# reonaledo/Multi-modality-Self-supervision

Hardware: AMD Instinct MI355X
Metric: image-text pairs/sec pretraining step, BERT-base seq512 (higher is better)
Workload: dtype f16

## Files before the change

### include/medvill.h

```cpp
#ifndef MEDVILL_H_
#define MEDVILL_H_

#include <stddef.h>
#include <stdint.h>

#ifdef __cplusplus
extern "C" {
#endif

#define MV_ABI_VERSION 6

enum { MV_F32 = 0, MV_BF16 = 1, MV_F16 = 2 };

enum {
  MV_OK = 0,
  MV_E_ARG = -1,
  MV_E_SHAPE = -2,
  MV_E_DTYPE = -3,
  MV_E_WORKSPACE = -4,
  MV_E_NO_RCCL = -5,
  MV_E_COMM_BASE = -1000
};

enum {
// ... 27 lines not shown

size_t mv_gemm_workspace_bytes(int dtype, int ta, int tb, int M, int N, int K);
size_t mv_workspace_bytes(int hidden, int intermediate, int vocab, int img_hidden, int max_rows, int max_label_rows, int max_regions);

typedef struct mv_group_problem {
  const void* A; const void* B; void* C;
  int lda, ldb, ldc;
  int No, Ko, rows;
} mv_group_problem;
size_t mv_gemm_grouped_table_bytes(int count);
int mv_gemm_grouped_fill(int dtype, int count, const mv_group_problem* problems, int n_blocks, void* table_host, size_t table_bytes);
size_t mv_gemm_grouped_workspace_bytes(const void* table_host);
int mv_gemm_grouped_decode(const void* table_host, int unit, int* out);
int mv_gemm_grouped_tn(int dtype, int count, const void* table_host, const void* table_dev, float* ws, size_t ws_bytes,
                       int accumulate, const float* alpha_dev, void* stream);

int mv_mask_pack(const int64_t* mask, int mask_ndim, int B, int L,
                 uint32_t* bits, uint8_t* tileinfo, void* stream);

int mv_mask_build(const int32_t* desc, int B, int L, uint32_t* bits, uint8_t* tileinfo, void* stream);

int mv_mlm_draws(unsigned long long key, int B, int S, int vocab, float* u, int32_t* rnd, void* stream);
int mv_mlm_corrupt(const int64_t* ids, const int32_t* lengths, const float* u, const int32_t* rnd, const int32_t* family,
                   int B, int N, int S, int64_t* input_txt, int64_t* segment, int64_t* txt_labels, int32_t* n_ids,
                   int32_t* desc, int32_t* counts, int32_t* label_rows, int32_t* label_ids, int32_t* n_labels, void* stream);

int mv_mask_verify_host(const int64_t* mask, int mask_ndim, const int32_t* desc, int B, int L, int threads, long long* first_mismatch);

int mv_comm_unique_id(void* id128);
int mv_comm_init(void** comm_out, int rank, int world, const void* id128);
// ... 142 lines not shown
```

### multi-modality-self-supervision_amd/_lib.py

```python
from __future__ import annotations

import ctypes as C
import os

import torch

HERE = os.path.dirname(os.path.abspath(__file__))
LIB_PATH = os.environ.get("MV_LIB_PATH") or os.path.join(HERE, "libmedvill_hip.so")
DBG_LIB_PATH = os.environ.get("MV_DBG_LIB_PATH") or (LIB_PATH[:-3] + "_dbg.so")

MV_F32, MV_BF16, MV_F16 = 0, 1, 2
EPI_NONE, EPI_BIAS, EPI_BIAS_GELU, EPI_BIAS_RES, EPI_DGELU, EPI_RES, EPI_BIAS_TANH, EPI_BIAS_GELU_D, EPI_MUL, EPI_BIAS_RELU, EPI_BIAS_RES_RELU = range(11)
_ERR = {-1: "MV_E_ARG (null pointer / bad size)", -2: "MV_E_SHAPE (unsupported shape or alignment)",
        -3: "MV_E_DTYPE", -4: "MV_E_WORKSPACE (workspace too small)", -5: "MV_E_NO_RCCL (librccl could not be loaded)"}

vp, i32, i64, f32, sz, u64, f64 = C.c_void_p, C.c_int, C.c_longlong, C.c_float, C.c_size_t, C.c_ulonglong, C.c_double

PROTOTYPES = {
    "mv_abi_version": [],
    "mv_build_info": [],
    "mv_stream_create_cumask": [vp, i32, C.POINTER(C.c_void_p)],
    "mv_stream_destroy": [vp],
    "mv_comm_unique_id": [vp],
    "mv_comm_init": [C.POINTER(C.c_void_p), i32, i32, vp],
    "mv_comm_allreduce_async": [vp, vp, sz, i32, vp],
    "mv_comm_wait": [vp, vp],
    "mv_comm_destroy": [vp],
    "mv_gemm": [i32, i32, i32, i32, i32, i32, vp, i32, vp, i32, vp, i32, i32, vp, i32, vp, i32, i32, vp, i32, vp, i32, i32,
                i32, vp, sz, i32, f32, u64, vp, vp, vp],
    "mv_gemm_workspace_bytes": [i32, i32, i32, i32, i32, i32],
    "mv_workspace_bytes": [i32, i32, i32, i32, i32, i32, i32],
    "mv_gemm_grouped_table_bytes": [i32],
    "mv_gemm_grouped_fill": [i32, i32, vp, i32, vp, sz],
    "mv_gemm_grouped_workspace_bytes": [vp],
    "mv_gemm_grouped_decode": [vp, i32, C.POINTER(C.c_int)],
    "mv_gemm_grouped_tn": [i32, i32, vp, vp, vp, sz, i32, vp, vp],
    "mv_mask_pack": [vp, i32, i32, i32, vp, vp, vp],
    "mv_mask_build": [vp, i32, i32, vp, vp, vp],
    "mv_mask_verify_host": [vp, i32, vp, i32, i32, i32, C.POINTER(C.c_longlong)],
    "mv_mlm_draws": [u64, i32, i32, i32, vp, vp, vp],
    "mv_mlm_corrupt": [vp, vp, vp, vp, vp, i32, i32, i32, vp, vp, vp, vp, vp, vp, vp, vp, vp, vp],
    "mv_pack_plan": [vp, i32, i32, vp, vp, vp, vp],
    "mv_tail_perm": [vp, i32, i32, vp, i32, vp, vp, vp, vp, vp],
    "mv_attn_fwd": [i32, vp, vp, vp, vp, vp, vp, i32, i32, i32, i32, f32, vp, vp, i32, vp, vp],
    "mv_attn_dropmask": [f32, u64, i32, i32, i32, vp, vp, vp],
    "mv_attn_bwd": [i32, vp, vp, vp, vp, vp, vp, vp, vp, i32, i32, i32, i32, f32, vp, vp, i32, vp, vp],
    "mv_layernorm_fwd": [i32, vp, i32, vp, vp, vp, vp, vp, vp, i32, i32, f32, vp],
    "mv_layernorm_bwd": [i32, vp, vp, i32, vp, vp, vp, vp, vp, vp, vp, i32, i32, vp, f32, u64, vp, vp],
    "mv_embed_fwd": [i32, vp, vp, vp, vp, vp, vp, vp, vp, vp, vp, vp, vp, vp, vp, vp, vp, i32, i32, i32, i32, i32, i32, f32, f32, f32,
                     u64, vp, i32, vp],
    "mv_embed_bwd": [i32, vp, vp, vp, vp, vp, vp, vp, vp, vp, vp, vp, vp, vp, vp, vp, vp, i32, i32, i32, i32, i32, i32, i32, f32, f32,
# ... 26 lines not shown
    "mv_bce_fwd_bwd": [vp, i32, vp, vp, i32, i32, vp, vp, i32, i32, vp, f32, vp, vp, vp, vp],
    "mv_rows_mul": [i32, vp, i32, vp, vp, i32, vp, i32, i32, vp, i32, vp],
    "mv_tensor_sqnorms": [vp, sz, vp, i32, vp, i32, vp, vp, vp],
    "mv_bce_multilabel": [vp, i32, vp, vp, i32, i32, vp, vp, i32, i32, vp, f32, vp, vp, vp, vp],
    "mv_bertadam_step": [vp, vp, vp, vp, vp, vp, sz, vp, i32, vp, i32, vp, f64, f64, f64, f32, f32, f32, i32, i32, f64, i32, vp, vp],
    "mv_lm_loss_fwd": [vp, i32, i32, i32, vp, vp, i32, f64, vp, vp, vp, vp],
    "mv_lm_loss_select": [vp, vp, vp, vp, i32, i32, i32, vp, vp, vp, vp],
    "mv_lm_loss_bwd": [vp, i32, i32, i32, vp, vp, vp, vp, i32, f64, vp, vp, vp, vp, vp, vp, i32, i32, vp],
    "mv_pair_draws": [u64, u64, i32, i32, vp, vp],
    "mv_pair_negatives": [vp, i32, i32, vp, u64, u64, vp, i32, vp, vp, vp],
    "mv_pair_assemble": [vp, vp, i32, vp, i32, i32, vp, vp, i32, i32, i32, i32, vp, vp, vp, vp, vp, vp, vp],
    "mv_rank_groups": [vp, vp, i32, i32, vp, i32, vp, vp, vp, vp, vp],
}
DEBUG_PROTOTYPES = {"mv_debug_set_knob": [i32, i32], "mv_debug_get_knob": [i32]}
_RESTYPE = {"mv_build_info": C.c_char_p, "mv_gemm_workspace_bytes": C.c_size_t, "mv_workspace_bytes": C.c_size_t,
            "mv_gemm_grouped_table_bytes": C.c_size_t, "mv_gemm_grouped_workspace_bytes": C.c_size_t}
ABI_VERSION = 6

KNOBS = {"impl": (0, 0), "gemm_force": (1, 0), "gemm_nj": (2, 0), "gemm_dbg": (3, 0), "attn_planes": (4, 16), "persistent_cus": (5, 0),
         "rowops_variant": (6, 0), "attn_order": (7, 0), "attn_fwd": (8, 0), "gemm_rounds": (9, 1)}

_lib = None
_dbg = None
_knobs = {k: d for k, (_, d) in KNOBS.items()}


def _open(path, protos):
    lib = C.CDLL(path)
    for name, args in protos.items():
        fn = getattr(lib, name)
        fn.argtypes = args
# ... 89 lines not shown
```

### multi-modality-self-supervision_amd/csrc/mv_gemm.hip

```cpp
#include "mv_gemm_common.h"
#include "mv_gemm_group.h"

#define GT_BM 128
#define GT_BN 128
#define GT_BK 64
#define GT_STAGE_BYTES 32768

template <bool TR>
__device__ __forceinline__ void stage_load(u32x4 (&reg)[4], __amdgpu_buffer_rsrc_t rs, unsigned bytes, int ld,
                                           int row0, int rows_total, int k0, int kend, int tid) {
#pragma unroll
  for (int i = 0; i < 4; ++i) {
    const int idx = tid + 256 * i;
    unsigned off;
    bool ok;
    if (!TR) {
      const int r = idx >> 3, ch = idx & 7;
      const int gr = row0 + r, gk = k0 + ch * 8;
      ok = (gr < rows_total) && (gk < kend);
      off = ((unsigned)gr * (unsigned)ld + (unsigned)gk) * 2u;
    } else {
      const int kr = idx >> 4, ch = idx & 15;
      const int gk = k0 + kr, gc = row0 + ch * 8;
      ok = (gk < kend) && (gc < rows_total);
// ... 539 lines not shown
  if (n_blocks < 0) return MV_E_ARG;
  return mv_group_fill(dtype, count, problems, n_blocks > 0 ? n_blocks : grouped_blocks(), table_host, table_bytes);
}

extern "C" size_t mv_gemm_grouped_workspace_bytes(const void* table_host) { return mv_group_workspace_bytes(table_host); }

extern "C" int mv_gemm_grouped_decode(const void* table_host, int unit, int* out) {
  if (!table_host || !out) return MV_E_ARG;
  const MvGroupHeader& h = *(const MvGroupHeader*)table_host;
  if (h.magic != MV_GROUP_MAGIC || unit < 0 || unit >= h.direct + h.tail * h.split) return MV_E_ARG;
  const MvGroupUnit d = mv_group_decode(h, (const MvGroupEntry*)((const char*)table_host + sizeof(MvGroupHeader)), unit);
  out[0] = d.problem; out[1] = d.m0; out[2] = d.n0; out[3] = d.kbeg; out[4] = d.kend; out[5] = d.slice; out[6] = d.tile;
  return MV_OK;
}

extern "C" int mv_gemm_grouped_tn(int dtype, int count, const void* table_host, const void* table_dev, float* ws, size_t ws_bytes,
                                  int accumulate, const float* alpha_dev, void* stream_) {
  if (!table_host || !table_dev || count <= 0) return MV_E_ARG;
  const int rc = mv_group_check_table(dtype, count, table_host);
  if (rc != MV_OK) return rc;
  if (g_mv_impl != 0) return MV_E_DTYPE;
  if (((uintptr_t)table_dev) & 15) return MV_E_SHAPE;
  const MvGroupHeader& h = *(const MvGroupHeader*)table_host;
  const size_t need = mv_group_workspace_bytes(table_host);
  if (need > 0 && (!ws || ws_bytes < need || (((uintptr_t)ws) & 15))) return MV_E_WORKSPACE;
  GroupArgs ga;
  ga.table = table_dev; ga.ws = ws; ga.alpha = alpha_dev; ga.accumulate = accumulate;
  const int n_blk = h.n_blocks < grouped_blocks() ? h.n_blocks : grouped_blocks();
  return mv_launch_ring_tn_grouped(h, ga, dtype == MV_F16, n_blk, (hipStream_t)stream_);
}

extern "C" int mv_conv2d(int dtype, const void* x, const void* w, void* y, int y_dtype, int B, int H, int W, int C, int O, int kh, int kw,
                         int stride, int pad, const float* bias, int epi, const void* R, int r_dtype, void* stream_) {
  hipStream_t stream = (hipStream_t)stream_;
  if (!x || !w || !y || B <= 0 || H <= 0 || W <= 0 || C <= 0 || O <= 0 || kh <= 0 || kw <= 0 || stride <= 0 || pad < 0) return MV_E_ARG;
  if (dtype != MV_BF16 || g_mv_impl != 0) return MV_E_DTYPE;
  if (y_dtype != MV_F32 && y_dtype != MV_BF16) return MV_E_DTYPE;
  if (epi != MV_EPI_NONE && epi != MV_EPI_BIAS && epi != MV_EPI_BIAS_RELU && epi != MV_EPI_BIAS_RES_RELU) return MV_E_ARG;
  if (epi != MV_EPI_NONE && !bias) return MV_E_ARG;
  if (epi == MV_EPI_BIAS_RES_RELU && (!R || (r_dtype != MV_F32 && r_dtype != MV_BF16))) return MV_E_ARG;
  if ((C & 7) || (C & (C - 1)) || (O & 3)) return MV_E_SHAPE;
  const int Ho = (H + 2 * pad - kh) / stride + 1, Wo = (W + 2 * pad - kw) / stride + 1;
  if (Ho <= 0 || Wo <= 0) return MV_E_SHAPE;
  const long long rows = (long long)B * Ho * Wo;
// ... 28 lines not shown
```

### multi-modality-self-supervision_amd/csrc/mv_gemm_group.h

```cpp
#pragma once
#include <stddef.h>
#include <stdint.h>
#include "../../include/medvill.h"

#if defined(__HIPCC__)
#include <hip/hip_runtime.h>
#define MV_HD __host__ __device__ __forceinline__
#else
#define MV_HD inline
#endif

#define MV_GROUP_MAGIC 0x4d564754
#define MV_GROUP_MAX_PROBLEMS 256
#define MV_GROUP_MAX_SPLIT 8
#define MV_GROUP_TILE 256
#define MV_GROUP_BK 64

struct MvGroupHeader {
  int magic, count, dtype, n_blocks;
  int units;
  int direct;
  int tail;
  int split;
  int pad[8];
};
struct MvGroupEntry {
  const void* A; const void* B; void* C;
  int lda, ldb, ldc;
  int M, N, K;
  unsigned bytesA, bytesB;
  int unit0;
  int kchunk;
};
struct GroupArgs {
  const void* table;
  float* ws;
  const float* alpha;
  int accumulate;
};
static_assert(sizeof(MvGroupHeader) == 64 && sizeof(MvGroupEntry) == 64, "table layout");

MV_HD int mv_group_tiles(int M, int N) { return ((M + MV_GROUP_TILE - 1) / MV_GROUP_TILE) * ((N + MV_GROUP_TILE - 1) / MV_GROUP_TILE); }

MV_HD int mv_group_tail_split(int R, int G) {
  if (R <= 0 || G <= 0) return 1;
  for (int s = 1; s <= MV_GROUP_MAX_SPLIT; ++s) {
    const long long n = (long long)R * s, rounds = (n + G - 1) / G;
    if (10 * n >= 7 * rounds * G) return s;
  }
  return 1;
}

MV_HD int mv_group_xcd_remap(int u, int n) {
// ... 119 lines not shown
    if (e[i].bytesA != mv_group_operand_bytes(e[i].K, e[i].lda, e[i].M) || e[i].bytesB != mv_group_operand_bytes(e[i].K, e[i].ldb, e[i].N)) return MV_E_ARG;
    if (e[i].unit0 != u0 || e[i].kchunk <= 0 || (e[i].kchunk % MV_GROUP_BK) != 0 || (long long)e[i].kchunk * h.split < e[i].K) return MV_E_ARG;
    u0 += mv_group_tiles(e[i].M, e[i].N);
  }
  const int rem = h.units % h.n_blocks;
  if (h.units != u0 || h.split != mv_group_tail_split(rem, h.n_blocks) || h.tail != (h.split > 1 ? rem : 0) || h.direct != h.units - h.tail) return MV_E_ARG;
  return 0;
}

inline size_t mv_group_workspace_bytes(const void* table) {
  if (!table) return 0;
  const MvGroupHeader& h = *(const MvGroupHeader*)table;
  if (h.magic != MV_GROUP_MAGIC || h.tail <= 0 || h.split <= 1) return 0;
  return (size_t)h.tail * h.split * MV_GROUP_TILE * MV_GROUP_TILE * sizeof(float);
}
#endif
```

### multi-modality-self-supervision_amd/csrc/mv_gemm_ring.h

```cpp
#pragma once
#include "mv_gemm_common.h"
#include "mv_gemm_group.h"

template <bool TA, bool TB, bool BP512, int NJ, int KS, bool F16>
__device__ __forceinline__ void g2_stage_mma_tr(const char* tA, const char* tB, int wm, int wn, int l15, int lq, f32x4 (&acc)[8][NJ]) {
#pragma unroll
  for (int ks = 0; ks < KS; ++ks) {
    bf16x8 fb[NJ];
#pragma unroll
    for (int j = 0; j < NJ; ++j) fb[j] = g2_frag<TB, BP512, KS>(tB, wn + j * 16, l15, lq, ks);
    bf16x8 cur = g2_frag<TA, true, KS>(tA, wm, l15, lq, ks);
#pragma unroll
    for (int i = 0; i < 8; ++i) {
      bf16x8 nxt = cur;
      if (i + 1 < 8) nxt = g2_frag<TA, true, KS>(tA, wm + (i + 1) * 16, l15, lq, ks);
      __builtin_amdgcn_sched_barrier(0);
#pragma unroll
      for (int j = 0; j < NJ; ++j) acc[i][j] = mma16<F16>(fb[j], cur, acc[i][j]);
      __builtin_amdgcn_sched_barrier(0);
      cur = nxt;
    }
  }
}

template <bool TA, bool TB, int NJ, int WN, int NSTAGE, int KS, bool F16 = false, int MI = 8>
__global__ __launch_bounds__(128 * WN, 2) void gemm_ring_kernel(GemmArgs p) {
  extern __shared__ __attribute__((aligned(16))) char smem[];
  constexpr int NW = 2 * WN;
  constexpr int BN = WN * 16 * NJ;
  constexpr bool BP512 = BN > 128;
  constexpr int BKS = G2_BK * KS;
  constexpr int BM = 32 * MI;
  constexpr int A_BYTES = BM * 64 * KS;
// ... 265 lines not shown
  constexpr int BN = WN * 16 * NJ;
  constexpr bool BP512 = BN > 128;
  constexpr int BKS = G2_BK * KS;
  constexpr int A_BYTES = 16384 * KS;
  constexpr int B_BYTES = (BP512 ? 16384 : 8192) * KS;
  constexpr int STAGE = A_BYTES + B_BYTES;
  constexpr int LPS = STAGE / 1024 / NW;
  constexpr int EPI_OPS = 28;
  static_assert(BN == MV_GROUP_TILE && G2_BM == MV_GROUP_TILE && BKS == MV_GROUP_BK, "the table's units are 256 x 256 tiles, 64-deep stages");
  static_assert(NW * 4608 <= STAGE, "epilogue scratch must fit in one ring stage");
  static_assert((NSTAGE - 2) * LPS + EPI_OPS < 64, "vmcnt is a 6-bit counter");
  const int tid = threadIdx.x, lane = tid & 63;
  const int wid = __builtin_amdgcn_readfirstlane(tid >> 6);
  const int l15 = lane & 15, lq = lane >> 4;
  const int wm = (wid / WN) * 128, wn = (wid % WN) * (16 * NJ);
  const int G = gridDim.x;
  const MvGroupHeader h = group_header(ga.table);
  const group_tab_t tab = (group_tab_t)((uintptr_t)ga.table + sizeof(MvGroupHeader));

  int iu = blockIdx.x, is = 0, im0 = 0, in0 = 0, ik0 = 0, ikend = 0, inst = 0, ilda = 0, ildb = 0, iM = 0, iN = 0;
  unsigned ibA = 0, ibB = 0;
  dma_rsrc_t rsA = {0, 0, 0, 0}, rsB = {0, 0, 0, 0};
  unsigned ifs = 0, cfs = 0;
  auto issue_unit = [&]() {
    const MvGroupUnit d = mv_group_decode(h, tab, iu);
    const group_tab_t e = tab + d.problem;
    im0 = d.m0; in0 = d.n0; ik0 = d.kbeg; ikend = d.kend;
    inst = max(1, (d.kend - d.kbeg + BKS - 1) / BKS);
    ilda = e->lda; ildb = e->ldb; iM = e->M; iN = e->N; ibA = e->bytesA; ibB = e->bytesB;
    rsA = dma_rsrc(e->A, ibA);
// ... 12 lines not shown
      if (iu < units) issue_unit();
    }
  };
#pragma unroll
  for (int i = 0; i < NSTAGE - 1; ++i) issue_one();

  int epi_ops = 0;
  for (int cu = blockIdx.x; cu < units; cu += G) {
    const MvGroupUnit d = mv_group_decode(h, tab, cu);
    const int nst = max(1, (d.kend - d.kbeg + BKS - 1) / BKS);
    f32x4 acc[8][NJ];
#pragma unroll
    for (int i = 0; i < 8; ++i)
#pragma unroll
      for (int j = 0; j < NJ; ++j) acc[i][j] = (f32x4){0.f, 0.f, 0.f, 0.f};

    for (int s = 0; s < nst; ++s) {
      const int younger = (int)(ifs - cfs) - 1;
      const bool after_epi = (s == 0) && epi_ops > 0;
      if (after_epi) {
        if (NSTAGE > 2 && younger >= 1) wait_vmcnt<(NSTAGE > 2 ? LPS : 0) + EPI_OPS>();
        else wait_vmcnt<EPI_OPS>();
      } else {
        if (NSTAGE > 2 && younger >= 1) wait_vmcnt<(NSTAGE > 2 ? LPS : 0)>();
        else wait_vmcnt<0>();
      }
      __builtin_amdgcn_s_barrier();
      __builtin_amdgcn_sched_barrier(0);
      issue_one();
      const char* tA = smem + (cfs % NSTAGE) * STAGE;
      const char* tB = tA + A_BYTES;
      g2_stage_mma_tr<TA, TB, BP512, NJ, KS, F16>(tA, tB, wm, wn, l15, lq, acc);
      ++cfs;
    }

    __builtin_amdgcn_s_barrier();
    char* scr = smem + ((cfs + NSTAGE - 1) % NSTAGE) * STAGE + wid * 4608;
    const int rrow = lane >> 4, c4 = lane & 15;
    const bool col_on = (c4 * 4) < 16 * NJ;
    constexpr int G2_NI = 8;
    GemmArgs p = {};
    p.c_dtype = MV_F32; p.epi = MV_EPI_NONE; p.alpha = ga.alpha; p.accumulate = ga.accumulate;
    if (d.slice >= 0) {
      p.M = MV_GROUP_TILE; p.N = MV_GROUP_TILE; p.splitk = h.split;
      p.ws = ga.ws + (size_t)(d.tile - h.direct) * h.split * (MV_GROUP_TILE * MV_GROUP_TILE);
      const int split = d.slice, m0 = 0, n0 = 0;
      G2_EPI_BODY(-1)
      epi_ops = EPI_OPS;
// ... 38 lines not shown
```

### multi-modality-self-supervision_amd/csrc/mv_gemm_ring_tn.hip

```cpp
#include "mv_gemm_ring.h"

int mv_launch_ring_tn(const GemmArgs& p, bool f16, int variant, int tiles, int splitk, int n_cu, hipStream_t stream) {
  dim3 grid(tiles, splitk);
  if (f16) {
    if (variant == 2) LAUNCH_RING(true, true, 4, 2, 3, 1, true);
    else if (variant == 24) LAUNCH_PRING(true, true, 4, 4, 2, true);
    else LAUNCH_RING(true, true, 4, 4, 2, 2, true);
  } else {
    if (variant == 24) LAUNCH_PRING(true, true, 4, 4, 2, false);
    else LAUNCH_RING(true, true, 4, 4, 2, 2, false);
  }
  return MV_OK;
}

__global__ __launch_bounds__(256) void splitk_reduce_grouped_kernel(GroupArgs ga) {
  const MvGroupHeader h = group_header(ga.table);
  const group_tab_t tab = (group_tab_t)((uintptr_t)ga.table + sizeof(MvGroupHeader));
  const int tile = h.direct + blockIdx.x;
  const group_tab_t e = tab + mv_group_find(tab, h.count, tile);
  int m0, n0;
  mv_group_raster(tile - e->unit0, e->M, e->N, m0, n0);
  const int M = e->M, N = e->N, ldc = e->ldc;
  float* C = (float*)e->C;
  const int nsl = (e->K + e->kchunk - 1) / e->kchunk;
// ... 3 lines not shown
  const int c = (threadIdx.x & 63) * 4, n = n0 + c;
  for (int r = blockIdx.y * 16 + (threadIdx.x >> 6); r < blockIdx.y * 16 + 16; r += 4) {
    const int m = m0 + r;
    if (m >= M || n >= N) continue;
    f32x4 s = {0.f, 0.f, 0.f, 0.f};
    for (int k = 0; k < nsl; ++k) s += *(const f32x4*)(slab + ((size_t)k * MV_GROUP_TILE + r) * MV_GROUP_TILE + c);
    s *= al;
    float* dst = C + (size_t)m * ldc + n;
    if (vec) {
      if (ga.accumulate) s += *(const f32x4*)dst;
      *(f32x4*)dst = s;
    } else {
      for (int j = 0; j < 4 && n + j < N; ++j) dst[j] = ga.accumulate ? dst[j] + s[j] : s[j];
    }
  }
}

int mv_launch_ring_tn_grouped(const MvGroupHeader& h, const GroupArgs& ga, bool f16, int n_blk, hipStream_t stream) {
  constexpr size_t shm = (size_t)2 * 2 * (16384 + 16384);
  static bool attr_set = false;
  if (!attr_set) {
    (void)hipFuncSetAttribute((const void*)gemm_pring_grouped_kernel<4, 4, 2, true>, hipFuncAttributeMaxDynamicSharedMemorySize, (int)shm);
    (void)hipFuncSetAttribute((const void*)gemm_pring_grouped_kernel<4, 4, 2, false>, hipFuncAttributeMaxDynamicSharedMemorySize, (int)shm);
    attr_set = true;
  }
  const int units = h.direct + h.tail * h.split;
  const dim3 grid(units < n_blk ? units : n_blk), block(512);
  if (f16) hipLaunchKernelGGL((gemm_pring_grouped_kernel<4, 4, 2, true>), grid, block, shm, stream, ga, units);
  else hipLaunchKernelGGL((gemm_pring_grouped_kernel<4, 4, 2, false>), grid, block, shm, stream, ga, units);
  MV_CHECK_LAUNCH();
// ... 7 lines not shown
```

### multi-modality-self-supervision_amd/engine.py

```python
from __future__ import annotations

import math
import os
from collections import OrderedDict
from dataclasses import asdict, dataclass

import torch

from . import hip_ops as ops
from ._lib import (EPI_BIAS, EPI_BIAS_GELU, EPI_BIAS_GELU_D, EPI_BIAS_RES, EPI_BIAS_TANH, EPI_MUL, EPI_NONE, EPI_RES, MV_BF16, MV_F16,
                   MV_F32)


@dataclass
class ModelConfig:
    vocab_size: int = 30522
    hidden: int = 768
    layers: int = 12
    heads: int = 12
    intermediate: int = 3072
    max_pos: int = 512
    type_vocab: int = 2
    img_hidden: int = 2048
    ln_eps: float = 1e-12
# ... 133 lines not shown
            self.scaler = torch.zeros(8, dtype=torch.float32, device=self.device)
            self.reset_scaler()
        self.shadow_dirty = True
        self._ws = {}
        self._gemm_ws = {}
        self._side = None
        self.training = False
        self.keep_acts = True
        self.ln_in_16 = os.environ.get("MV_LN_IN_16", "1") != "0"
        self.dz_nt = os.environ.get("MV_DZ_NT", "1") != "0"
        self._w2t, self._w2t_ev, self._w2t_stale = None, None, True
        self.head_on_side = True
        self.fused_colsum = os.environ.get("MV_FUSED_COLSUM", "1") != "0"
        self.grouped_dw = os.environ.get("MV_GROUPED_DW", "1") != "0"
        self.grouped_dw_parts = max(0, int(os.environ.get("MV_GROUPED_DW_PARTS", "0")))
        self._dw_group = {}
        self.head_params_on_side = True
        self.late_opt_wait = True
        self.itm_on_side = True
        self.logits_16 = os.environ.get("MV_LOGITS_16", "0") == "1"
        self.tail_queries = os.environ.get("MV_TAIL_QUERIES", "1") != "0"
        self._mask_stream = None
        self._dE_ev = None
        self._opt_ev = None
        self.head_splitk = True
        self.dw_splitk = 0
        self.drop_seed = (torch.initial_seed() ^ 0x5DEECE66D) & 0xFFFFFFFFFFFFFFFF
        self.drop_counter = 0
        self._bind()

# ... 583 lines not shown
        def side_done():
            ev = torch.cuda.Event()
            ev.record(side)
            return ev

        if bucket_hook:
            bucket_hook("heads", side_done() if side is not main else None)
        use_w2t = self.dz_nt and self.is16
        mfma_on = self.fused_colsum and self.is16 and ops.get_impl() == 0
        if use_w2t:
            if self._w2t_stale or self._w2t is None:
                self.refresh_w2t(on_side=False)
            main.wait_event(self._w2t_ev)
        pd, dk = S["p_drop"], S["drop_keys"]
        group = [] if (self.grouped_dw and bucket_hook is None and self.is16 and ops.get_impl() == 0 and H % 8 == 0 and I % 8 == 0) else None

        def dW(defer, dy_, x_, gW_, No, Ko, rows, lda, ldb):
            if defer:
                group.append((dy_, x_, gW_, No, Ko, rows, lda, ldb, Ko))
            else:
                fork()
                with torch.cuda.stream(side):
                    self._dW(dy_, x_, gW_, No, Ko, rows, lda=lda, ldb=ldb)

        full = [l for l in reversed(range(cfg.layers)) if S["layers"][l]["rows"] == M]
        parts = min(self.grouped_dw_parts or (len(full) + 1) // 2, max(len(full), 1))
        flush_after = {full[(len(full) * (i + 1) + parts - 1) // parts - 1]: i for i in range(parts)} if (group is not None and full) else {}

        def flush(part):
            shared = {t.data_ptr() for t in (dctx, da, dxb[0], dxb[1])} | {self._ws[k].data_ptr() for k in ("bw_dctx_tail", "bw_dx_unperm") if k in self._ws}
# ... 20 lines not shown
            tail = a_["rows"] != M_all
            M = a_["rows"]
            dpre2 = self._buf(f"bw_dpre2_{l}", (M, H), adt)
            dprd2 = self._buf(f"bw_dprd2_{l}", (M, H), adt) if pd > 0 else None
            dpre1 = self._buf(f"bw_dpre1_{l}", (M, H), adt)
            dprd1 = self._buf(f"bw_dprd1_{l}", (M, H), adt) if pd > 0 else None
            dz = self._buf(f"bw_dz_{l}", (M, I), adt)
            dqkv = self._buf(f"bw_dqkv_{l}", (M_all, 3 * H), adt)
            ops.layernorm_bwd(dy, a_["pre2"], a_["mean2"], a_["rstd2"], self.p[p + "output.LayerNorm.weight"], dpre2,
                              g[p + "output.LayerNorm.weight"], g[p + "output.LayerNorm.bias"], g[p + "output.dense.bias"], M, H,
                              dx_drop=dprd2, p_drop=pd, drop_key=dk[(self.SITE_OUT2, l)], unscale=us)
            dproj2 = dprd2 if dprd2 is not None else dpre2
            defer = group is not None and not tail
            dW(defer, dproj2, a_["i"], g[p + "output.dense.weight"], H, I, M, H, I)
            dz_part = None
            if use_w2t and mfma_on and M >= 256 and I >= 1024 and I % 256 == 0 and ((M + 255) // 256) * ((I + 127) // 128) >= 128:
                dz_part = self._buf(f"bw_dzpart_{l}", (2 * ((M + 255) // 256), I), torch.float32)
            if use_w2t:
                ops.gemm(dproj2, self._w2t[l], dz, M=M, N=I, K=H, epi=EPI_MUL, r=a_["dgelu"], colsum_part=dz_part)
            else:
                ops.gemm(dproj2, self.w[p + "output.dense.weight"], dz, tb=True, M=M, N=I, K=H, epi=EPI_MUL, r=a_["dgelu"])
            fork()
            with torch.cuda.stream(side):
                if dz_part is not None:
                    ops.colsum_partials(dz_part, dz_part.shape[0], I, I, g[p + "intermediate.dense.bias"], unscale=us)
                else:
                    ops.colsum(dz, I, M, I, g[p + "intermediate.dense.bias"], accumulate=True, unscale=us)
                if defer:
                    group.append((dz, a_["a"], g[p + "intermediate.dense.weight"], I, H, M, I, H, H))
                else:
                    self._dW(dz, a_["a"], g[p + "intermediate.dense.weight"], I, H, M, lda=I, ldb=H)
            ops.gemm(dz, self.w[p + "intermediate.dense.weight"], da, tb=True, M=M, N=H, K=I, epi=EPI_RES, r=dpre2)
            ops.layernorm_bwd(da, a_["pre1"], a_["mean1"], a_["rstd1"], self.p[p + "attention.output.LayerNorm.weight"], dpre1,
                              g[p + "attention.output.LayerNorm.weight"], g[p + "attention.output.LayerNorm.bias"],
                              g[p + "attention.output.dense.bias"], M, H, dx_drop=dprd1, p_drop=pd,
                              drop_key=dk[(self.SITE_OUT1, l)], unscale=us)
            dproj1 = dprd1 if dprd1 is not None else dpre1
            dW(defer, dproj1, a_["ctx_tail"] if tail else a_["ctx"], g[p + "attention.output.dense.weight"], H, H, M, H, H)
            if tail:
                dctx_s = self._buf("bw_dctx_tail", (M, H), adt)
                ops.gemm(dproj1, self.w[p + "attention.output.dense.weight"], dctx_s, tb=True, M=M, N=H, K=H)
                dctx.zero_()
                ops.scatter_rows(dctx_s, H, S["sel"] if S["tq"] is None else S["tq"][3], M, H, dctx, H, accumulate=False)
            else:
                ops.gemm(dproj1, self.w[p + "attention.output.dense.weight"], dctx, tb=True, M=M, N=H, K=H)
            M = M_all
            tq = S["tq"] if tail else None
            ops.attn_bwd(a_["qkv"], a_["ctx"], dctx, a_["lse"], S["bits"], S["tinfo"], dqkv, delta, B, Lq, A, dh, cu=S["cu"],
                         total_rows=M, p_drop=pd, dropbits=a_["dropbits"], qlim=tq[2] if tq is not None else None)
            fork()
            with torch.cuda.stream(side):
                ops.colsum(dqkv, 3 * H, M, 3 * H, gbqkv, accumulate=True, unscale=us)
                if defer:
                    group.append((dqkv, a_["x"], gWqkv, 3 * H, H, M, 3 * H, H, H))
                    if l in flush_after:
                        flush(flush_after[l])
                else:
                    self._dW(dqkv, a_["x"], gWqkv, 3 * H, H, M, lda=3 * H, ldb=H)
                ev_layer = side_done()
            dx = dxb[l & 1]
            if tail:
                ops.gemm(dqkv, Wqkv, dx, tb=True, M=M, N=H, K=3 * H)
                ops.scatter_rows(dpre1, H, S["sel"] if tq is None else tq[3], a_["rows"], H, dx, H, accumulate=True)
                if tq is not None:
                    dxu = self._buf("bw_dx_unperm", (M, H), adt)
                    ops.scatter_rows(dx, H, tq[0], M, H, dxu, H, accumulate=False)
                    dx = dxu
            else:
                ops.gemm(dqkv, Wqkv, dx, tb=True, M=M, N=H, K=3 * H, epi=EPI_RES, r=dpre1)
# ... 86 lines not shown
```

### multi-modality-self-supervision_amd/hip_ops.py

```python
from __future__ import annotations

import ctypes

import torch

from . import _lib as L
from ._lib import (EPI_BIAS, EPI_BIAS_GELU, EPI_BIAS_GELU_D, EPI_BIAS_RELU, EPI_BIAS_RES, EPI_BIAS_RES_RELU, EPI_BIAS_TANH, EPI_DGELU,
                   EPI_MUL, EPI_NONE, EPI_RES, MV_BF16, MV_F16,
                   MV_F32)


def _lib():
    return L.load()


def gemm(a, b, c, *, ta=False, tb=False, M, N, K, lda=None, ldb=None, ldc=None, bias=None, epi=EPI_NONE, r=None, ldr=None,
         c2=None, ldc2=None, c3=None, ldc3=None, splitk=1, ws=None, accumulate=False, p_drop=0.0, drop_key=0, alpha=None, colsum_part=None):
    L.require_cuda(a, b, c, bias, r, c2, c3, ws, alpha, colsum_part)
    if colsum_part is not None and (colsum_part.dtype != torch.float32 or colsum_part.numel() < 2 * ((M + 255) // 256) * N):
        raise ValueError("colsum_part: f32 [2*ceil(M/256), N]")
    lda = lda if lda is not None else (M if ta else K)
    ldb = ldb if ldb is not None else (N if tb else K)
    ldc = ldc if ldc is not None else N
    ldr = ldr if ldr is not None else N
# ... 430 lines not shown


class GroupedTN:

    def __init__(self, device):
        self.device = torch.device(device)
        self.key = None
        self.count = 0
        self.dtype = 0
        self.host = None
        self.dev = None
        self.staged = None
        self.staged_ev = None
        self.uploads = 0
        self.launches = 0

    def set(self, dtype, problems, n_blocks=0):
        dt = dtype if isinstance(dtype, int) else L.dt_of(torch.empty(0, dtype=dtype))
        key = (dt, int(n_blocks), L.get_knob("persistent_cus"),
               tuple((a.data_ptr(), b.data_ptr(), c.data_ptr(), No, Ko, rows, lda, ldb, ldc) for a, b, c, No, Ko, rows, lda, ldb, ldc in problems))
        if key == self.key:
            return False
        for a, b, c, *_ in problems:
            L.require_cuda(a, b, c)
            if L.dt_of(a) != dt or L.dt_of(b) != dt or c.dtype != torch.float32:
                raise TypeError("grouped dW: 16-bit operands of one encoding, f32 outputs")
        n = len(problems)
        arr = (GroupProblem * max(n, 1))(*[GroupProblem(k[0], k[1], k[2], k[6], k[7], k[8], k[3], k[4], k[5]) for k in key[3]])
        nbytes = int(_lib().mv_gemm_grouped_table_bytes(n))
        host = self.host if self.host is not None and len(self.host) >= nbytes else ctypes.create_string_buffer(max(nbytes, 1))
        self.key = None
        L.check(_lib().mv_gemm_grouped_fill(dt, n, arr, int(n_blocks), host, nbytes), f"mv_gemm_grouped_fill(count={n})")
        if self.staged is None or self.staged.numel() < nbytes:
            self.staged = torch.empty(nbytes, dtype=torch.uint8).pin_memory()
            self.dev = torch.empty(nbytes, dtype=torch.uint8, device=self.device)
        elif self.staged_ev is not None:
            self.staged_ev.synchronize()
        ctypes.memmove(self.staged.data_ptr(), host, nbytes)
        self.dev[:nbytes].copy_(self.staged[:nbytes], non_blocking=True)
        self.staged_ev = torch.cuda.Event()
        self.staged_ev.record()
        self.host, self.key, self.count, self.dtype = host, key, n, dt
        self.uploads += 1
        return True

    def workspace_bytes(self) -> int:
        return int(_lib().mv_gemm_grouped_workspace_bytes(self.host))

    def units(self):
        hdr = (ctypes.c_int * 16).from_buffer(self.host)
        out = (ctypes.c_int * 7)()
        res = []
        for u in range(hdr[5] + hdr[6] * hdr[7]):
            L.check(_lib().mv_gemm_grouped_decode(self.host, u, out), "mv_gemm_grouped_decode")
            res.append(tuple(out))
        return res

    def launch(self, ws=None, accumulate=False, alpha=None):
        L.require_cuda(ws, alpha)
        rc = _lib().mv_gemm_grouped_tn(self.dtype, self.count, self.host, L.ptr(self.dev), L.ptr(ws), (ws.numel() * 4) if ws is not None else 0,
                                       int(accumulate), L.ptr(alpha), L.stream_ptr())
        L.check(rc, f"mv_gemm_grouped_tn(count={self.count})")
        self.launches += 1


def set_gemm_variant(force: int = 0, nj: int = 0):
    L.set_knob("gemm_force", int(force) & 0xff)
    L.set_knob("gemm_nj", int(nj))
    L.set_knob("gemm_dbg", int(force) >> 8)


def gemm_rows(x, w, c, *, M, N, K, ldx=None, ldw=None, ldc=None, bias=None, epi=EPI_NONE, r=None, ldr=None):
    L.require_cuda(x, w, c, bias, r)
    if x.dtype != w.dtype:
        raise TypeError("gemm_rows operands must share a dtype")
    if bias is not None and bias.dtype != torch.float32:
        raise TypeError("bias must be f32")
# ... 289 lines not shown
```

Baseline: 2836.

## Fuse bias-gradient column sums into grouped dW GEMM kernel

Bias-gradient column sums for the deferred QKV and intermediate weight gradients are now computed inside the grouped TN dW kernel. Each wave accumulates dot-with-ones of the A fragments it already loads for the MMA, with split-K partials reduced in the tail kernel. This removes separate colsum launches and extra reads of dz/dqkv on the side stream. In exchange it adds fdot2 work to the MMA inner loop, more register pressure, and a bigger table upload. The bias gradient of deferred layers also now waits for the grouped launch instead of being computed early.

```diff
diff --git a/include/medvill.h b/include/medvill.h
--- a/include/medvill.h
+++ b/include/medvill.h
@@ -65,6 +65,9 @@
 int mv_gemm_grouped_decode(const void* table_host, int unit, int* out);
 int mv_gemm_grouped_tn(int dtype, int count, const void* table_host, const void* table_dev, float* ws, size_t ws_bytes,
                        int accumulate, const float* alpha_dev, void* stream);
+size_t mv_gemm_grouped_colsum_workspace_bytes(const void* table_host);
+int mv_gemm_grouped_tn_colsum(int dtype, int count, const void* table_host, const void* table_dev, float* const* colsum_dev,
+                              float* ws, size_t ws_bytes, int accumulate, const float* alpha_dev, void* stream);
 
 int mv_mask_pack(const int64_t* mask, int mask_ndim, int B, int L,
                  uint32_t* bits, uint8_t* tileinfo, void* stream);
diff --git a/multi-modality-self-supervision_amd/_lib.py b/multi-modality-self-supervision_amd/_lib.py
--- a/multi-modality-self-supervision_amd/_lib.py
+++ b/multi-modality-self-supervision_amd/_lib.py
@@ -35,6 +35,8 @@
     "mv_gemm_grouped_workspace_bytes": [vp],
     "mv_gemm_grouped_decode": [vp, i32, C.POINTER(C.c_int)],
     "mv_gemm_grouped_tn": [i32, i32, vp, vp, vp, sz, i32, vp, vp],
+    "mv_gemm_grouped_colsum_workspace_bytes": [vp],
+    "mv_gemm_grouped_tn_colsum": [i32, i32, vp, vp, vp, vp, sz, i32, vp, vp],
     "mv_mask_pack": [vp, i32, i32, i32, vp, vp, vp],
     "mv_mask_build": [vp, i32, i32, vp, vp, vp],
     "mv_mask_verify_host": [vp, i32, vp, i32, i32, i32, C.POINTER(C.c_longlong)],
@@ -91,7 +93,8 @@
 }
 DEBUG_PROTOTYPES = {"mv_debug_set_knob": [i32, i32], "mv_debug_get_knob": [i32]}
 _RESTYPE = {"mv_build_info": C.c_char_p, "mv_gemm_workspace_bytes": C.c_size_t, "mv_workspace_bytes": C.c_size_t,
-            "mv_gemm_grouped_table_bytes": C.c_size_t, "mv_gemm_grouped_workspace_bytes": C.c_size_t}
+            "mv_gemm_grouped_table_bytes": C.c_size_t, "mv_gemm_grouped_workspace_bytes": C.c_size_t,
+            "mv_gemm_grouped_colsum_workspace_bytes": C.c_size_t}
 ABI_VERSION = 6
 
 KNOBS = {"impl": (0, 0), "gemm_force": (1, 0), "gemm_nj": (2, 0), "gemm_dbg": (3, 0), "attn_planes": (4, 16), "persistent_cus": (5, 0),
diff --git a/multi-modality-self-supervision_amd/csrc/mv_gemm.hip b/multi-modality-self-supervision_amd/csrc/mv_gemm.hip
--- a/multi-modality-self-supervision_amd/csrc/mv_gemm.hip
+++ b/multi-modality-self-supervision_amd/csrc/mv_gemm.hip
@@ -577,20 +577,36 @@
   return MV_OK;
 }
 
-extern "C" int mv_gemm_grouped_tn(int dtype, int count, const void* table_host, const void* table_dev, float* ws, size_t ws_bytes,
-                                  int accumulate, const float* alpha_dev, void* stream_) {
+extern "C" size_t mv_gemm_grouped_colsum_workspace_bytes(const void* table_host) { return mv_group_colsum_workspace_bytes(table_host); }
+
+static int grouped_tn(int dtype, int count, const void* table_host, const void* table_dev, float* const* colsum_dev, float* ws, size_t ws_bytes,
+                      int accumulate, const float* alpha_dev, void* stream_) {
   if (!table_host || !table_dev || count <= 0) return MV_E_ARG;
   const int rc = mv_group_check_table(dtype, count, table_host);
   if (rc != MV_OK) return rc;
   if (g_mv_impl != 0) return MV_E_DTYPE;
   if (((uintptr_t)table_dev) & 15) return MV_E_SHAPE;
   const MvGroupHeader& h = *(const MvGroupHeader*)table_host;
-  const size_t need = mv_group_workspace_bytes(table_host);
+  if (((uintptr_t)colsum_dev) & 7) return MV_E_SHAPE;
+  const size_t slabs = mv_group_workspace_bytes(table_host);
+  const size_t need = slabs + (colsum_dev ? mv_group_colsum_workspace_bytes(table_host) : 0);
   if (need > 0 && (!ws || ws_bytes < need || (((uintptr_t)ws) & 15))) return MV_E_WORKSPACE;
   GroupArgs ga;
   ga.table = table_dev; ga.ws = ws; ga.alpha = alpha_dev; ga.accumulate = accumulate;
+  ga.csum = colsum_dev; ga.cws = (colsum_dev && ws) ? ws + slabs / sizeof(float) : nullptr;
   const int n_blk = h.n_blocks < grouped_blocks() ? h.n_blocks : grouped_blocks();
   return mv_launch_ring_tn_grouped(h, ga, dtype == MV_F16, n_blk, (hipStream_t)stream_);
+}
+
+extern "C" int mv_gemm_grouped_tn(int dtype, int count, const void* table_host, const void* table_dev, float* ws, size_t ws_bytes,
+                                  int accumulate, const float* alpha_dev, void* stream_) {
+  return grouped_tn(dtype, count, table_host, table_dev, nullptr, ws, ws_bytes, accumulate, alpha_dev, stream_);
+}
+
+extern "C" int mv_gemm_grouped_tn_colsum(int dtype, int count, const void* table_host, const void* table_dev, float* const* colsum_dev,
+                                         float* ws, size_t ws_bytes, int accumulate, const float* alpha_dev, void* stream_) {
+  if (!colsum_dev) return MV_E_ARG;
+  return grouped_tn(dtype, count, table_host, table_dev, colsum_dev, ws, ws_bytes, accumulate, alpha_dev, stream_);
 }
 
 extern "C" int mv_conv2d(int dtype, const void* x, const void* w, void* y, int y_dtype, int B, int H, int W, int C, int O, int kh, int kw,
diff --git a/multi-modality-self-supervision_amd/csrc/mv_gemm_group.h b/multi-modality-self-supervision_amd/csrc/mv_gemm_group.h
--- a/multi-modality-self-supervision_amd/csrc/mv_gemm_group.h
+++ b/multi-modality-self-supervision_amd/csrc/mv_gemm_group.h
@@ -37,6 +37,8 @@
   float* ws;
   const float* alpha;
   int accumulate;
+  const void* csum;
+  float* cws;
 };
 static_assert(sizeof(MvGroupHeader) == 64 && sizeof(MvGroupEntry) == 64, "table layout");
 
@@ -186,4 +188,11 @@
   if (h.magic != MV_GROUP_MAGIC || h.tail <= 0 || h.split <= 1) return 0;
   return (size_t)h.tail * h.split * MV_GROUP_TILE * MV_GROUP_TILE * sizeof(float);
 }
+
+inline size_t mv_group_colsum_workspace_bytes(const void* table) {
+  if (!table) return 0;
+  const MvGroupHeader& h = *(const MvGroupHeader*)table;
+  if (h.magic != MV_GROUP_MAGIC || h.tail <= 0 || h.split <= 1) return 0;
+  return (size_t)h.tail * h.split * MV_GROUP_TILE * sizeof(float);
+}
 #endif
diff --git a/multi-modality-self-supervision_amd/csrc/mv_gemm_ring.h b/multi-modality-self-supervision_amd/csrc/mv_gemm_ring.h
--- a/multi-modality-self-supervision_amd/csrc/mv_gemm_ring.h
+++ b/multi-modality-self-supervision_amd/csrc/mv_gemm_ring.h
@@ -2,8 +2,29 @@
 #include "mv_gemm_common.h"
 #include "mv_gemm_group.h"
 
-template <bool TA, bool TB, bool BP512, int NJ, int KS, bool F16>
-__device__ __forceinline__ void g2_stage_mma_tr(const char* tA, const char* tB, int wm, int wn, int l15, int lq, f32x4 (&acc)[8][NJ]) {
+template <bool F16>
+__device__ __forceinline__ float g2_frag_sum(bf16x8 f, float c) {
+  typedef __attribute__((ext_vector_type(2))) _Float16 h2_t;
+  typedef __attribute__((ext_vector_type(2))) __bf16 b2_t;
+  if constexpr (F16) {
+    const f16x8 h = __builtin_bit_cast(f16x8, f);
+    const h2_t one = {(_Float16)1.0f, (_Float16)1.0f};
+    c = __builtin_amdgcn_fdot2(__builtin_shufflevector(h, h, 0, 1), one, c, false);
+    c = __builtin_amdgcn_fdot2(__builtin_shufflevector(h, h, 2, 3), one, c, false);
+    c = __builtin_amdgcn_fdot2(__builtin_shufflevector(h, h, 4, 5), one, c, false);
+    c = __builtin_amdgcn_fdot2(__builtin_shufflevector(h, h, 6, 7), one, c, false);
+  } else {
+    const b2_t one = __builtin_bit_cast(b2_t, 0x3f803f80u);
+    c = __builtin_amdgcn_fdot2_f32_bf16(__builtin_shufflevector(f, f, 0, 1), one, c, false);
+    c = __builtin_amdgcn_fdot2_f32_bf16(__builtin_shufflevector(f, f, 2, 3), one, c, false);
+    c = __builtin_amdgcn_fdot2_f32_bf16(__builtin_shufflevector(f, f, 4, 5), one, c, false);
+    c = __builtin_amdgcn_fdot2_f32_bf16(__builtin_shufflevector(f, f, 6, 7), one, c, false);
+  }
+  return c;
+}
+template <bool TA, bool TB, bool BP512, int NJ, int KS, bool F16, bool CS = false>
+__device__ __forceinline__ void g2_stage_mma_tr(const char* tA, const char* tB, int wm, int wn, int l15, int lq, f32x4 (&acc)[8][NJ],
+                                                float* cs = nullptr, int cown = 0) {
 #pragma unroll
   for (int ks = 0; ks < KS; ++ks) {
     bf16x8 fb[NJ];
@@ -17,6 +38,13 @@
       __builtin_amdgcn_sched_barrier(0);
 #pragma unroll
       for (int j = 0; j < NJ; ++j) acc[i][j] = mma16<F16>(fb[j], cur, acc[i][j]);
+      if constexpr (CS) {
+        if ((i >> 1) == cown) {
+          float c = cs[i & 1];
+          asm volatile("" : "+v"(c));
+          cs[i & 1] = g2_frag_sum<F16>(cur, c);
+        }
+      }
       __builtin_amdgcn_sched_barrier(0);
       cur = nxt;
     }
@@ -312,6 +340,7 @@
   const int wid = __builtin_amdgcn_readfirstlane(tid >> 6);
   const int l15 = lane & 15, lq = lane >> 4;
   const int wm = (wid / WN) * 128, wn = (wid % WN) * (16 * NJ);
+  const int cown = wid % WN;
   const int G = gridDim.x;
   const MvGroupHeader h = group_header(ga.table);
   const group_tab_t tab = (group_tab_t)((uintptr_t)ga.table + sizeof(MvGroupHeader));
@@ -354,6 +383,11 @@
     for (int i = 0; i < 8; ++i)
 #pragma unroll
       for (int j = 0; j < NJ; ++j) acc[i][j] = (f32x4){0.f, 0.f, 0.f, 0.f};
+    const __attribute__((address_space(4))) uint64_t* ctab = (const __attribute__((address_space(4))) uint64_t*)(uintptr_t)ga.csum;
+    int cw = -1;
+    if (ga.csum && d.n0 == 0 && ctab[d.problem] != 0) cw = cown;
+    cw = __builtin_amdgcn_readfirstlane(cw);
+    float cs[2] = {0.f, 0.f};
 
     for (int s = 0; s < nst; ++s) {
       const int younger = (int)(ifs - cfs) - 1;
@@ -370,8 +404,29 @@
       issue_one();
       const char* tA = smem + (cfs % NSTAGE) * STAGE;
       const char* tB = tA + A_BYTES;
-      g2_stage_mma_tr<TA, TB, BP512, NJ, KS, F16>(tA, tB, wm, wn, l15, lq, acc);
+      g2_stage_mma_tr<TA, TB, BP512, NJ, KS, F16, true>(tA, tB, wm, wn, l15, lq, acc, cs, cw);
       ++cfs;
+    }
+
+    if (cw >= 0) {
+      float* cdst = (float*)(uintptr_t)ctab[d.problem];
+      const int cM = tab[d.problem].M;
+      const float al = ga.alpha ? *ga.alpha : 1.0f;
+#pragma unroll
+      for (int f = 0; f < 2; ++f) {
+        float v = cs[f];
+        v += __shfl_xor(v, 16, 64);
+        v += __shfl_xor(v, 32, 64);
+        const int r = wm + (2 * cown + f) * 16 + l15;
+        if (lq == 0) {
+          if (d.slice >= 0) ga.cws[((size_t)(d.tile - h.direct) * h.split + d.slice) * MV_GROUP_TILE + r] = v;
+          else if (d.m0 + r < cM) {
+            v *= al;
+            if (ga.accumulate) v += cdst[d.m0 + r];
+            cdst[d.m0 + r] = v;
+          }
+        }
+      }
     }
 
     __builtin_amdgcn_s_barrier();
diff --git a/multi-modality-self-supervision_amd/csrc/mv_gemm_ring_tn.hip b/multi-modality-self-supervision_amd/csrc/mv_gemm_ring_tn.hip
--- a/multi-modality-self-supervision_amd/csrc/mv_gemm_ring_tn.hip
+++ b/multi-modality-self-supervision_amd/csrc/mv_gemm_ring_tn.hip
@@ -41,6 +41,17 @@
       for (int j = 0; j < 4 && n + j < N; ++j) dst[j] = ga.accumulate ? dst[j] + s[j] : s[j];
     }
   }
+  if (ga.csum && n0 == 0 && blockIdx.y == 0) {
+    float* cd = (float*)(uintptr_t)((const __attribute__((address_space(4))) uint64_t*)(uintptr_t)ga.csum)[(int)(e - tab)];
+    const int m = m0 + (int)threadIdx.x;
+    if (cd && m < M) {
+      const float* part = ga.cws + (size_t)blockIdx.x * h.split * MV_GROUP_TILE + threadIdx.x;
+      float t = 0.f;
+      for (int k = 0; k < nsl; ++k) t += part[(size_t)k * MV_GROUP_TILE];
+      t *= al;
+      cd[m] = ga.accumulate ? cd[m] + t : t;
+    }
+  }
 }
 
 int mv_launch_ring_tn_grouped(const MvGroupHeader& h, const GroupArgs& ga, bool f16, int n_blk, hipStream_t stream) {
diff --git a/multi-modality-self-supervision_amd/engine.py b/multi-modality-self-supervision_amd/engine.py
--- a/multi-modality-self-supervision_amd/engine.py
+++ b/multi-modality-self-supervision_amd/engine.py
@@ -171,6 +171,7 @@
         self.fused_colsum = os.environ.get("MV_FUSED_COLSUM", "1") != "0"
         self.grouped_dw = os.environ.get("MV_GROUPED_DW", "1") != "0"
         self.grouped_dw_parts = max(0, int(os.environ.get("MV_GROUPED_DW_PARTS", "0")))
+        self.grouped_colsum = os.environ.get("MV_GROUPED_COLSUM", "1") != "0"
         self._dw_group = {}
         self.head_params_on_side = True
         self.late_opt_wait = True
@@ -784,6 +785,7 @@
             main.wait_event(self._w2t_ev)
         pd, dk = S["p_drop"], S["drop_keys"]
         group = [] if (self.grouped_dw and bucket_hook is None and self.is16 and ops.get_impl() == 0 and H % 8 == 0 and I % 8 == 0) else None
+        group_cs = group is not None and self.grouped_colsum
 
         def dW(defer, dy_, x_, gW_, No, Ko, rows, lda, ldb):
             if defer:
@@ -834,22 +836,26 @@
             defer = group is not None and not tail
             dW(defer, dproj2, a_["i"], g[p + "output.dense.weight"], H, I, M, H, I)
             dz_part = None
-            if use_w2t and mfma_on and M >= 256 and I >= 1024 and I % 256 == 0 and ((M + 255) // 256) * ((I + 127) // 128) >= 128:
+            cs_here = defer and group_cs
+            if not cs_here and use_w2t and mfma_on and M >= 256 and I >= 1024 and I % 256 == 0 and ((M + 255) // 256) * ((I + 127) // 128) >= 128:
                 dz_part = self._buf(f"bw_dzpart_{l}", (2 * ((M + 255) // 256), I), torch.float32)
             if use_w2t:
                 ops.gemm(dproj2, self._w2t[l], dz, M=M, N=I, K=H, epi=EPI_MUL, r=a_["dgelu"], colsum_part=dz_part)
             else:
                 ops.gemm(dproj2, self.w[p + "output.dense.weight"], dz, tb=True, M=M, N=I, K=H, epi=EPI_MUL, r=a_["dgelu"])
-            fork()
-            with torch.cuda.stream(side):
-                if dz_part is not None:
-                    ops.colsum_partials(dz_part, dz_part.shape[0], I, I, g[p + "intermediate.dense.bias"], unscale=us)
-                else:
-                    ops.colsum(dz, I, M, I, g[p + "intermediate.dense.bias"], accumulate=True, unscale=us)
-                if defer:
-                    group.append((dz, a_["a"], g[p + "intermediate.dense.weight"], I, H, M, I, H, H))
-                else:
-                    self._dW(dz, a_["a"], g[p + "intermediate.dense.weight"], I, H, M, lda=I, ldb=H)
+            if cs_here:
+                group.append((dz, a_["a"], g[p + "intermediate.dense.weight"], I, H, M, I, H, H, g[p + "intermediate.dense.bias"]))
+            else:
+                fork()
+                with torch.cuda.stream(side):
+                    if dz_part is not None:
+                        ops.colsum_partials(dz_part, dz_part.shape[0], I, I, g[p + "intermediate.dense.bias"], unscale=us)
+                    else:
+                        ops.colsum(dz, I, M, I, g[p + "intermediate.dense.bias"], accumulate=True, unscale=us)
+                    if defer:
+                        group.append((dz, a_["a"], g[p + "intermediate.dense.weight"], I, H, M, I, H, H))
+                    else:
+                        self._dW(dz, a_["a"], g[p + "intermediate.dense.weight"], I, H, M, lda=I, ldb=H)
             ops.gemm(dz, self.w[p + "intermediate.dense.weight"], da, tb=True, M=M, N=H, K=I, epi=EPI_RES, r=dpre2)
             ops.layernorm_bwd(da, a_["pre1"], a_["mean1"], a_["rstd1"], self.p[p + "attention.output.LayerNorm.weight"], dpre1,
                               g[p + "attention.output.LayerNorm.weight"], g[p + "attention.output.LayerNorm.bias"],
@@ -870,9 +876,10 @@
                          total_rows=M, p_drop=pd, dropbits=a_["dropbits"], qlim=tq[2] if tq is not None else None)
             fork()
             with torch.cuda.stream(side):
-                ops.colsum(dqkv, 3 * H, M, 3 * H, gbqkv, accumulate=True, unscale=us)
+                if not cs_here:
+                    ops.colsum(dqkv, 3 * H, M, 3 * H, gbqkv, accumulate=True, unscale=us)
                 if defer:
-                    group.append((dqkv, a_["x"], gWqkv, 3 * H, H, M, 3 * H, H, H))
+                    group.append((dqkv, a_["x"], gWqkv, 3 * H, H, M, 3 * H, H, H) + ((gbqkv,) if cs_here else ()))
                     if l in flush_after:
                         flush(flush_after[l])
                 else:
diff --git a/multi-modality-self-supervision_amd/hip_ops.py b/multi-modality-self-supervision_amd/hip_ops.py
--- a/multi-modality-self-supervision_amd/hip_ops.py
+++ b/multi-modality-self-supervision_amd/hip_ops.py
@@ -468,23 +468,39 @@
         self.staged_ev = None
         self.uploads = 0
         self.launches = 0
-
-    def set(self, dtype, problems, n_blocks=0):
+        self.csum_off = None
+
+    def set(self, dtype, problems, n_blocks=0, colsum=None):
         dt = dtype if isinstance(dtype, int) else L.dt_of(torch.empty(0, dtype=dtype))
+        dests = [q[9] if len(q) > 9 else None for q in problems]
+        if colsum is not None:
+            if len(colsum) != len(problems):
+                raise ValueError("grouped dW: one column-sum destination (or None) per problem")
+            dests = [d if d is not None else e for d, e in zip(colsum, dests)]
+        problems = [tuple(q[:9]) for q in problems]
         key = (dt, int(n_blocks), L.get_knob("persistent_cus"),
-               tuple((a.data_ptr(), b.data_ptr(), c.data_ptr(), No, Ko, rows, lda, ldb, ldc) for a, b, c, No, Ko, rows, lda, ldb, ldc in problems))
+               tuple((a.data_ptr(), b.data_ptr(), c.data_ptr(), No, Ko, rows, lda, ldb, ldc) for a, b, c, No, Ko, rows, lda, ldb, ldc in problems),
+               tuple(d.data_ptr() if d is not None else 0 for d in dests) if any(d is not None for d in dests) else None)
         if key == self.key:
             return False
         for a, b, c, *_ in problems:
             L.require_cuda(a, b, c)
             if L.dt_of(a) != dt or L.dt_of(b) != dt or c.dtype != torch.float32:
                 raise TypeError("grouped dW: 16-bit operands of one encoding, f32 outputs")
+        for d, q in zip(dests, problems):
+            if d is not None:
+                L.require_cuda(d)
+                if d.dtype != torch.float32 or d.numel() < q[3] or not d.is_contiguous():
+                    raise TypeError("grouped dW: a column-sum destination is a contiguous f32 [No]")
         n = len(problems)
         arr = (GroupProblem * max(n, 1))(*[GroupProblem(k[0], k[1], k[2], k[6], k[7], k[8], k[3], k[4], k[5]) for k in key[3]])
-        nbytes = int(_lib().mv_gemm_grouped_table_bytes(n))
+        tbytes = int(_lib().mv_gemm_grouped_table_bytes(n))
+        nbytes = tbytes + (8 * n if key[4] is not None else 0)
         host = self.host if self.host is not None and len(self.host) >= nbytes else ctypes.create_string_buffer(max(nbytes, 1))
         self.key = None
-        L.check(_lib().mv_gemm_grouped_fill(dt, n, arr, int(n_blocks), host, nbytes), f"mv_gemm_grouped_fill(count={n})")
+        L.check(_lib().mv_gemm_grouped_fill(dt, n, arr, int(n_blocks), host, tbytes), f"mv_gemm_grouped_fill(count={n})")
+        if key[4] is not None:
+            ctypes.memmove(ctypes.addressof(host) + tbytes, (ctypes.c_uint64 * n)(*key[4]), 8 * n)
         if self.staged is None or self.staged.numel() < nbytes:
             self.staged = torch.empty(nbytes, dtype=torch.uint8).pin_memory()
             self.dev = torch.empty(nbytes, dtype=torch.uint8, device=self.device)
@@ -495,11 +511,15 @@
         self.staged_ev = torch.cuda.Event()
         self.staged_ev.record()
         self.host, self.key, self.count, self.dtype = host, key, n, dt
+        self.csum_off = tbytes if key[4] is not None else None
         self.uploads += 1
         return True
 
     def workspace_bytes(self) -> int:
-        return int(_lib().mv_gemm_grouped_workspace_bytes(self.host))
+        nb = int(_lib().mv_gemm_grouped_workspace_bytes(self.host))
+        if self.csum_off is not None:
+            nb += int(_lib().mv_gemm_grouped_colsum_workspace_bytes(self.host))
+        return nb
 
     def units(self):
         hdr = (ctypes.c_int * 16).from_buffer(self.host)
@@ -512,9 +532,15 @@
 
     def launch(self, ws=None, accumulate=False, alpha=None):
         L.require_cuda(ws, alpha)
-        rc = _lib().mv_gemm_grouped_tn(self.dtype, self.count, self.host, L.ptr(self.dev), L.ptr(ws), (ws.numel() * 4) if ws is not None else 0,
-                                       int(accumulate), L.ptr(alpha), L.stream_ptr())
-        L.check(rc, f"mv_gemm_grouped_tn(count={self.count})")
+        ws_bytes = (ws.numel() * 4) if ws is not None else 0
+        if self.csum_off is not None:
+            rc = _lib().mv_gemm_grouped_tn_colsum(self.dtype, self.count, self.host, L.ptr(self.dev), self.dev.data_ptr() + self.csum_off, L.ptr(ws),
+                                                  ws_bytes, int(accumulate), L.ptr(alpha), L.stream_ptr())
+            L.check(rc, f"mv_gemm_grouped_tn_colsum(count={self.count})")
+        else:
+            rc = _lib().mv_gemm_grouped_tn(self.dtype, self.count, self.host, L.ptr(self.dev), L.ptr(ws), ws_bytes, int(accumulate), L.ptr(alpha),
+                                           L.stream_ptr())
+            L.check(rc, f"mv_gemm_grouped_tn(count={self.count})")
         self.launches += 1
 
 
```

Result: slower. 2710 (-4.4%).
